# PathologyFoundation/plip

Measured on NVIDIA H100. Metric: image-text pairs/sec (224x224, 77-tok), higher is better.
Workload: dtype bf16

## Files before the change

include/plip_b200.h:

```cpp
#ifndef PLIP_B200_H_
#define PLIP_B200_H_

#include <stdint.h>

#ifdef __cplusplus
extern "C" {
#endif

#define PLIP_API __attribute__((visibility("default")))

#define PLIP_B200_ABI_VERSION 5

#define PLIP_IMAGE_SIZE 224
#define PLIP_EMBED_DIM 512
#define PLIP_TEXT_SEQ 77
#define PLIP_VOCAB 49408

typedef struct plip_engine plip_engine_t;

enum plip_pixel_format {
  PLIP_PIX_F32_NCHW = 0,
  PLIP_PIX_BF16_NCHW = 1,
  PLIP_PIX_U8_NHWC = 2
};
// ... 130 lines not shown

typedef struct plip_densenet plip_densenet_t;
PLIP_API int plip_densenet_num_tensors(void);
PLIP_API int plip_densenet_tensor_info(int index, plip_tensor_info_t* info);
PLIP_API uint64_t plip_densenet_blob_bytes(void);
PLIP_API uint64_t plip_densenet_workspace_bytes(int max_micro_batch);
PLIP_API int plip_densenet_create(const void* host_blob, uint64_t blob_bytes, int device, int max_micro_batch,
                                  plip_densenet_t** out);
PLIP_API int plip_densenet_destroy(plip_densenet_t* e);
PLIP_API int plip_densenet_max_micro_batch(const plip_densenet_t* e);
PLIP_API int plip_densenet_encode(plip_densenet_t* e, const void* tiles_dev, int64_t n, float* out_dev, void* stream);

PLIP_API int plip_encode_images_host(plip_engine_t* e, const void* pixels_host, int pixel_format, int64_t n,
                                     float* out_host, int normalize);
PLIP_API int plip_encode_text_host(plip_engine_t* e, const void* ids_host, int ids_dtype,
                                   const void* attention_mask_host, int64_t n, int seq_len,
                                   float* out_host, int normalize);

typedef struct plip_kernel_time {
  char name[48];
  int32_t launches;
  float total_ms;
  double flops;
  double bytes;
} plip_kernel_time_t;
PLIP_API int plip_profile_enable(plip_engine_t* e, int on);
PLIP_API int plip_profile_read(plip_engine_t* e, plip_kernel_time_t* out, int cap, int* count);

PLIP_API int plip_dbg_set_operand_format(int operand_format);
PLIP_API int plip_dbg_gemm(const void* A_bf16, int lda, const void* W_bf16, int ldw, int M, int N, int K,
                           const float* bias, void* out, int ldo, const float* pos, int epilogue, int cluster_size,
                           int block_n, const float* colsum, const float* stats_in, int n_partials, void* xb_out,
                           float* stats_out, void* stream);
PLIP_API int plip_dbg_resize_filter(int in_size, int out_size, int xx, int32_t* k_host, int k_cap, int* xmin,
                                    int* count);
PLIP_API int plip_dbg_resize_filter_bilinear(int in_size, int out_size, int xx, int32_t* k_host, int k_cap, int* xmin,
                                             int* count);
PLIP_API int plip_dbg_text_bucket_plan(const int32_t* lens_host, int64_t n, int seq_len, int32_t* perm_host,
                                       int32_t* bucket_start_host, int32_t* bucket_prefix_host, int cap);
PLIP_API int plip_dbg_rowstats_cast(const float* x, int64_t rows, int dim, void* xb_bf16, float* stats, void* stream);
PLIP_API int plip_dbg_layernorm(const float* x, int64_t rows, int dim, int64_t in_row_stride,
                                const float* gamma, const float* beta, float* out_f32, void* out_bf16,
                                void* stream);
PLIP_API int plip_dbg_attention(const void* qkv_bf16, int64_t n_seq, int seq_len, int heads, int causal,
                                const int32_t* key_mask, void* out_bf16, void* stream);
PLIP_API int plip_dbg_attention_probs(const void* qkv_bf16, int64_t n_seq, int seq_len, int heads, int causal,
                                      const int32_t* key_mask, float* probs_dev, void* stream);
PLIP_API int plip_dbg_densenet_op(int op, const void* in_dev, int lda, int64_t n, int side, int c_in, const void* w_dev,
                                  const float* a_scale, const float* a_shift, const float* e_scale,
                                  const float* e_shift, void* out_dev, int ldo, void* stream);
PLIP_API int plip_dbg_im2col(const void* pixels, int pixel_format, int64_t n, void* out_bf16, void* stream);
PLIP_API int plip_dbg_pos_interp(const float* pos_dev, int grid_h, int grid_w, float* out_dev, void* stream);
PLIP_API int plip_dbg_hidden_states_hw(plip_engine_t* e, const void* pixels_dev, int pixel_format, int64_t n,
                                       int height, int width, int num_layers, float* hidden_dev, void* stream);
PLIP_API int plip_dbg_hidden_states(plip_engine_t* e, int tower, const void* input_dev, int input_format,
                                    const void* attention_mask_dev, int64_t n, int num_layers,
                                    float* hidden_dev, void* stream);

#ifdef __cplusplus
}
#endif
#endif
```

plip_b200/_lib.py:

```python
from __future__ import annotations

import ctypes as C
from pathlib import Path

_PKG = Path(__file__).resolve().parent
LIB_PATH = _PKG / "libplip_b200.so"

_vp = C.c_void_p
_i = C.c_int
_i64 = C.c_int64
_u64 = C.c_uint64
_f = C.c_float
_fp = C.c_void_p


class TensorInfo(C.Structure):

    _fields_ = [
        ("name", C.c_char * 96),
        ("offset", C.c_uint64),
        ("numel", C.c_uint64),
        ("dtype", C.c_int32),
        ("rows", C.c_int32),
        ("cols", C.c_int32),
# ... 22 lines not shown

class WarpDesc(C.Structure):

    _fields_ = [("affine", C.c_double * 6), ("perspective", C.c_double * 8), ("flip", C.c_int32),
                ("apply_perspective", C.c_int32), ("fill", C.c_int32), ("reserved", C.c_int32)]


class SgdProblem(C.Structure):

    _fields_ = [("alpha", C.c_double), ("pos_weight", C.c_double), ("neg_weight", C.c_double), ("pos_class", C.c_int32),
                ("sigma_index", C.c_int32)]


class TowerOutputs(C.Structure):

    _fields_ = [("embeds", C.c_void_p), ("pooled", C.c_void_p), ("last_hidden", C.c_void_p), ("hidden", C.c_void_p),
                ("attn", C.c_void_p), ("normalize", C.c_int32)]


SIGNATURES = {
    "plip_last_error": (C.c_char_p, []),
    "plip_abi_version": (_i, []),
    "plip_launch_count": (_u64, []),
    "plip_weights_num_tensors": (_i, []),
    "plip_weights_tensor_info": (_i, [_i, C.POINTER(TensorInfo)]),
    "plip_weights_blob_bytes": (_u64, []),
    "plip_create": (_i, [_vp, _u64, _f, _i, _i, C.POINTER(_vp)]),
    "plip_create_ex": (_i, [_vp, _u64, _f, _i, _i, _i, C.POINTER(_vp)]),
    "plip_operand_format": (_i, [_vp]),
    "plip_set_text_pooling": (_i, [_vp, _i]),
    "plip_set_last_layer_pruning": (_i, [_vp, _i]),
    "plip_last_layer_pruning": (_i, [_vp]),
    "plip_dbg_set_operand_format": (_i, [_i]),
    "plip_destroy": (_i, [_vp]),
    "plip_workspace_bytes": (_u64, [_i]),
    "plip_logit_scale_exp": (_f, [_vp]),
    "plip_max_micro_batch": (_i, [_vp]),
    "plip_encode_images": (_i, [_vp, _vp, _i, _i64, _fp, _i, _vp]),
    "plip_encode_images_hw": (_i, [_vp, _vp, _i, _i64, _i, _i, _fp, _i, _vp]),
    "plip_encode_windows": (_i, [_vp, _vp, _i, _i, _i64, _vp, _i64, _fp, _i, _vp]),
    "plip_window_background_counts": (_i, [_vp, _i, _i, _i64, _vp, _i64, _i, _vp, _vp]),
    "plip_encode_text": (_i, [_vp, _vp, _i, _vp, _i64, _i, _fp, _i, _vp]),
    "plip_encode_text_prefix": (_i, [_vp, _vp, _i, _vp, _i64, _i, _i, _fp, _i, _vp]),
    "plip_vision_outputs": (_i, [_vp, _vp, _i, _i64, _i, _i, C.POINTER(TowerOutputs), _vp]),
    "plip_text_outputs": (_i, [_vp, _vp, _i, _vp, _i64, _i, C.POINTER(TowerOutputs), _vp]),
    "plip_similarity": (_i, [_fp, _i64, _fp, _i64, _f, _i, _i, _fp, _i64, _vp]),
    "plip_similarity_topk": (_i, [_fp, _i64, _fp, _i64, _f, _i, _i, _i, _vp, _fp, _vp]),
    "plip_l2_normalize": (_i, [_fp, _i64, _i, _vp]),
    "plip_window_mask_counts": (_i, [_vp, _i, _i, _i, _i64, _vp, _i64, _i, _vp, _vp]),
    "plip_resize_crop_u8": (_i, [_vp, _u64, _vp, _i64, _vp, _vp]),
    "plip_resize_crop_bilinear_u8": (_i, [_vp, _u64, _vp, _i64, _vp, _vp]),
    "plip_warp_tiles_u8": (_i, [_vp, _vp, _vp, _i64, _vp]),
    "plip_resize_region_workspace": (_i, [_i, _i, _i, _i, _i, _i, C.POINTER(_u64)]),
    "plip_resize_region_u8": (_i, [_vp, _i64, _i, _i, _i, _i, _vp, _i64, _i, _i, _i, _i, _vp, _u64, _vp]),
    "plip_resize_filter_bounds": (_i, [_i, _i, _vp]),
    "plip_sgd_shuffle_permutation": (_i, [_i64, C.c_uint32, _vp]),
    "plip_sgd_workspace_bytes": (_i, [_i64, _i, _i, C.POINTER(_u64)]),
    "plip_sgd_fit": (_i, [_fp, _i64, _i, _vp, _i, _vp, _i, _vp, _i, _i, C.c_double, _i, _fp, _vp, _vp, _vp, _vp, _u64,
                          _vp]),
    "plip_linear_decision": (_i, [_fp, _i64, _i, _fp, _vp, _i, _fp, _vp, _vp]),
    "plip_densenet_num_tensors": (_i, []),
    "plip_densenet_tensor_info": (_i, [_i, C.POINTER(TensorInfo)]),
    "plip_densenet_blob_bytes": (_u64, []),
    "plip_densenet_workspace_bytes": (_u64, [_i]),
    "plip_densenet_create": (_i, [_vp, _u64, _i, _i, C.POINTER(_vp)]),
    "plip_densenet_destroy": (_i, [_vp]),
# ... 58 lines not shown
```

plip_b200/csrc/engine.cu:

```cuda
#include "kernels.cuh"

#include <stdlib.h>
#include <string.h>

#include <array>
#include <map>
#include <string>
#include <tuple>
#include <vector>

namespace plip {
const char* get_last_error();

namespace {

struct Spec {
  std::string name;
  int dtype;
  int rows, cols, fused;
  uint64_t offset, numel;
};

void add(std::vector<Spec>& v, const std::string& name, int dtype, int rows, int cols, int fused = 0) {
  Spec s;
// ... 1216 lines not shown
  }
  for (int k = 0; k < nb; ++k) {
    const int64_t r0 = start[k], cnt = start[k + 1] - start[k];
    if (cnt <= 0) continue;
    if (int rc = plip_encode_text_prefix(e, d_ids + (size_t)r0 * row_bytes, ids_dtype,
                                         d_mask ? d_mask + (size_t)r0 * row_bytes : nullptr, cnt, seq_len, prefix[k],
                                         e->d_out + r0 * kProj, normalize, e->s_compute)) return rc;
  }
  std::vector<float> tmp((size_t)n * kProj);
  PLIP_CUDA_CHECK(cudaMemcpyAsync(tmp.data(), e->d_out, (size_t)n * kProj * 4, cudaMemcpyDeviceToHost, e->s_compute));
  PLIP_CUDA_CHECK(cudaStreamSynchronize(e->s_compute));
  for (int64_t i = 0; i < n; ++i)
    memcpy(out_host + (size_t)perm[(size_t)i] * kProj, tmp.data() + (size_t)i * kProj, (size_t)kProj * 4);
  return 0;
}

PLIP_API int plip_dbg_text_bucket_plan(const int32_t* lens_host, int64_t n, int seq_len, int32_t* perm_host,
                                       int32_t* bucket_start_host, int32_t* bucket_prefix_host, int cap) {
  if (!lens_host || !bucket_start_host || !bucket_prefix_host || n <= 0 || seq_len < 1 || seq_len > kTxtSeq || cap < 1) {
    set_last_error("plip_dbg_text_bucket_plan: bad argument");
    return -2;
  }
  return plan_text_buckets(lens_host, n, seq_len, perm_host, bucket_start_host, bucket_prefix_host, cap);
}

static int g_dbg_f16 = 0;
PLIP_API int plip_dbg_set_operand_format(int operand_format) {
  PLIP_REQUIRE(operand_format == PLIP_OPERAND_BF16 || operand_format == PLIP_OPERAND_FP16,
               "plip_dbg_set_operand_format: unknown operand format %d", operand_format);
  g_dbg_f16 = operand_format == PLIP_OPERAND_FP16 ? 1 : 0;
  return 0;
}

PLIP_API int plip_dbg_gemm(const void* A_bf16, int lda, const void* W_bf16, int ldw, int M, int N, int K,
                           const float* bias, void* out, int ldo, const float* pos, int epilogue, int cluster_size,
                           int block_n, const float* colsum, const float* stats_in, int n_partials, void* xb_out,
                           float* stats_out, void* stream) {
  GemmArgs g;
  g.A = static_cast<const __nv_bfloat16*>(A_bf16); g.lda = lda;
  g.W = static_cast<const __nv_bfloat16*>(W_bf16); g.ldw = ldw;
  g.M = M; g.N = N; g.K = K;
  g.bias = bias; g.out = out; g.ldo = ldo; g.pos = pos; g.epi = epilogue;
  g.colsum = colsum; g.stats_in = reinterpret_cast<const float2*>(stats_in); g.n_partials = n_partials;
  g.xb_out = static_cast<__nv_bfloat16*>(xb_out); g.stats_out = reinterpret_cast<float2*>(stats_out);
  g.force_cg = cluster_size; g.force_bn = block_n;
  g.f16 = g_dbg_f16;
  return launch_gemm(g, static_cast<cudaStream_t>(stream));
}

PLIP_API int plip_dbg_rowstats_cast(const float* x, int64_t rows, int dim, void* xb_bf16, float* stats, void* stream) {
  return launch_rowstats_cast(x, rows, dim, static_cast<__nv_bfloat16*>(xb_bf16), reinterpret_cast<float2*>(stats),
                              g_dbg_f16, static_cast<cudaStream_t>(stream));
}

PLIP_API int plip_dbg_layernorm(const float* x, int64_t rows, int dim, int64_t in_row_stride, const float* gamma,
                                const float* beta, float* out_f32, void* out_bf16, void* stream) {
  return launch_layernorm(x, nullptr, in_row_stride, rows, dim, gamma, beta, out_f32,
                          static_cast<__nv_bfloat16*>(out_bf16), g_dbg_f16, static_cast<cudaStream_t>(stream));
}

PLIP_API int plip_dbg_attention(const void* qkv_bf16, int64_t n_seq, int seq_len, int heads, int causal,
                                const int32_t* key_mask, void* out_bf16, void* stream) {
  return launch_attention(static_cast<const __nv_bfloat16*>(qkv_bf16), n_seq, seq_len, heads, causal != 0, key_mask,
                          static_cast<__nv_bfloat16*>(out_bf16), g_dbg_f16, static_cast<cudaStream_t>(stream));
}

PLIP_API int plip_dbg_attention_probs(const void* qkv_bf16, int64_t n_seq, int seq_len, int heads, int causal,
                                      const int32_t* key_mask, float* probs_dev, void* stream) {
  return launch_attention_probs(static_cast<const __nv_bfloat16*>(qkv_bf16), n_seq, seq_len, heads, causal != 0,
                                key_mask, probs_dev, g_dbg_f16, static_cast<cudaStream_t>(stream));
}

PLIP_API int plip_dbg_im2col(const void* pixels, int pixel_format, int64_t n, void* out_bf16, void* stream) {
  return launch_im2col(pixels, pixel_format, n, kImage, kImage, static_cast<__nv_bfloat16*>(out_bf16), g_dbg_f16,
                       static_cast<cudaStream_t>(stream));
}

PLIP_API int plip_dbg_pos_interp(const float* pos_dev, int grid_h, int grid_w, float* out_dev, void* stream) {
// ... 18 lines not shown
```

plip_b200/csrc/gemm.cuh:

```cuda
#pragma once
#include "common.cuh"

namespace plip {

enum GemmEpilogue : int {
  EPI_BIAS_BF16 = 0,
  EPI_BIAS_GELU_BF16 = 1,
  EPI_BIAS_RESID_F32 = 2,
  EPI_PATCH_F32 = 3,
  EPI_F32 = 4,
  EPI_LN_BIAS_BF16 = 5,
  EPI_LN_BIAS_GELU_BF16 = 6,
  EPI_NULL = 7,
  EPI_SIM_F32 = 8,
  EPI_COUNT = 9
};

constexpr int kStatSlots = 8;

struct GemmArgs {
  const __nv_bfloat16* A = nullptr;
  int lda = 0;
  const __nv_bfloat16* W = nullptr;
  int ldw = 0;
  int M = 0, N = 0, K = 0;
  const float* bias = nullptr;
  const float* rowscale = nullptr;
  void* out = nullptr;
  int ldo = 0;
  const float* pos = nullptr;
  int patches = kPatches;
  int seq = kVisSeq;
  const float* colsum = nullptr;
  const float2* stats_in = nullptr;
  int n_partials = 0;
  __nv_bfloat16* xb_out = nullptr;
  float2* stats_out = nullptr;
  int* n_tiles_used = nullptr;
  int epi = EPI_F32;
  int f16 = 0;
  int force_cg = 0;
  int force_bn = 0;
};

int launch_gemm(const GemmArgs& g, cudaStream_t stream);

}
```

plip_b200/csrc/gemm_wgmma.cu:

```cuda
#include "gemm.cuh"
#include "wgmma.cuh"

#include <stdio.h>
#include <stdlib.h>

namespace plip {

namespace {

constexpr int BM = 64;
constexpr int BK = 64;
constexpr int kThreads = 288;
constexpr int kConsumerWarps = 8;
constexpr uint32_t A_STAGE = BM * BK * 2;
constexpr uint32_t kStoreStageBytes = 16 * 128;

constexpr int x_boxes(int BN, int EPI) {
  return EPI != EPI_BIAS_RESID_F32 ? 2 : BN == 192 ? 3 : 2;
}

template <int BN, int EPI>
struct Cfg {
  static constexpr uint32_t B_STAGE = BN * BK * 2;
  static constexpr uint32_t STAGE = A_STAGE + B_STAGE;
  static constexpr int XBOXES = x_boxes(BN, EPI);
  static constexpr uint32_t EPI_BYTES = kConsumerWarps * XBOXES * kStoreStageBytes;
  static constexpr uint32_t BAR_BYTES = EPI == EPI_BIAS_RESID_F32 ? 512 : 256;
  static constexpr uint32_t ALIGN_SLACK = 1024;
  static constexpr int kMaxStages = (227 * 1024 - BAR_BYTES - EPI_BYTES - ALIGN_SLACK) / STAGE;
  static constexpr int STAGES = kMaxStages > 8 ? 8 : kMaxStages;
  static constexpr uint32_t SMEM_BYTES = STAGES * STAGE + EPI_BYTES + BAR_BYTES + ALIGN_SLACK;
};

struct GemmDev {
  int M, N, K;
  const float* bias;
  const float* rowscale;
  void* out;
  int ldo;
  const float* pos;
  int patches, seq;
  const float* colsum;
  const float2* stats_in;
  int n_partials;
  __nv_bfloat16* xb_out;
  float2* stats_out;
};

template <bool F16, int BN>
__device__ __forceinline__ void wgmma_ss(float (&d)[BN / 2], uint64_t adesc, uint64_t bdesc, uint32_t scale_d) {
  if constexpr (BN == 128) wgmma_ss_n128<F16>(d, adesc, bdesc, scale_d);
  else if constexpr (BN == 192) wgmma_ss_n192<F16>(d, adesc, bdesc, scale_d);
  else wgmma_ss_n256<F16>(d, adesc, bdesc, scale_d);
}

__device__ __forceinline__ float2 ln_row_terms(const GemmDev& p, int grow) {
  float s1 = 0.f, s2 = 0.f;
#pragma unroll
  for (int j = 0; j < kStatSlots; ++j) {
    const float2 t = (grow < p.M && j < p.n_partials) ? __ldg(p.stats_in + static_cast<size_t>(grow) * kStatSlots + j)
                                                      : make_float2(0.f, 0.f);
    s1 += t.x;
    s2 += t.y;
  }
  const float inv_k = 1.0f / static_cast<float>(p.K);
  const float mean = s1 * inv_k;
  const float rstd = rsqrtf(fmaxf(s2 * inv_k - mean * mean, 0.f) + kLnEps);
  return make_float2(-rstd * mean, rstd);
}

template <int BN, int EPI, bool F16>
__device__ __forceinline__ void epilogue_warp(const GemmDev& p, const CUtensorMap* tmC, float (&d)[BN / 2], uint32_t stage_smem,
                                              uint32_t& stage_sel, uint32_t xbar, int row_base, int col_base, int n_blk, int lane,
                                              float2 ln0, float2 ln1) {
  constexpr bool LN_FOLD = (EPI == EPI_LN_BIAS_BF16 || EPI == EPI_LN_BIAS_GELU_BF16);
  constexpr bool GELU = (EPI == EPI_BIAS_GELU_BF16 || EPI == EPI_LN_BIAS_GELU_BF16);
  constexpr bool HAS_BIAS = (EPI == EPI_BIAS_BF16 || EPI == EPI_BIAS_GELU_BF16 || EPI == EPI_BIAS_RESID_F32 || LN_FOLD);
  constexpr bool OUT_BF16 = (EPI == EPI_BIAS_BF16 || EPI == EPI_BIAS_GELU_BF16 || LN_FOLD);
  const int q = lane & 3, rr = lane >> 2;
  const int row0 = row_base + rr, row1 = row0 + 8;

  if constexpr (EPI == EPI_NULL) {
    float acc = 0.f;
#pragma unroll
    for (int i = 0; i < BN / 2; ++i) acc += d[i];
    if (acc == 1.2345e30f && p.M < 0) reinterpret_cast<float*>(p.out)[0] = acc;
  } else if constexpr (OUT_BF16) {
#pragma unroll
    for (int blk = 0; blk < BN / 64; ++blk) {
      const uint32_t buf = stage_smem + (stage_sel & 1u) * kStoreStageBytes;
      ++stage_sel;
      if (lane == 0) tma_store_wait_read_but_one();
      __syncwarp();
#pragma unroll
      for (int jj = 0; jj < 8; ++jj) {
        const int j = blk * 8 + jj;
        const int col = col_base + 8 * j + 2 * q;
        const float2 b = __ldg(reinterpret_cast<const float2*>(p.bias + col));
        float v00 = d[4 * j + 0], v01 = d[4 * j + 1], v10 = d[4 * j + 2], v11 = d[4 * j + 3];
        if constexpr (LN_FOLD) {
          const float2 cs = __ldg(reinterpret_cast<const float2*>(p.colsum + col));
          v00 = fmaf(ln0.y, v00, fmaf(ln0.x, cs.x, b.x));
          v01 = fmaf(ln0.y, v01, fmaf(ln0.x, cs.y, b.y));
          v10 = fmaf(ln1.y, v10, fmaf(ln1.x, cs.x, b.x));
          v11 = fmaf(ln1.y, v11, fmaf(ln1.x, cs.y, b.y));
        } else {
          v00 += b.x; v01 += b.y; v10 += b.x; v11 += b.y;
        }
        if constexpr (GELU) {
          v00 = quick_gelu(v00); v01 = quick_gelu(v01); v10 = quick_gelu(v10); v11 = quick_gelu(v11);
        }
        st_shared_b32(buf + rr * 128 + ((jj ^ rr) << 4) + q * 4, pack_op2<F16>(v00, v01));
        st_shared_b32(buf + (rr + 8) * 128 + ((jj ^ rr) << 4) + q * 4, pack_op2<F16>(v10, v11));
      }
      fence_proxy_async_smem();
      __syncwarp();
      if (lane == 0) {
        tma_store_2d(tmC, buf, col_base + blk * 64, row_base);
        tma_store_commit();
      }
    }
  } else if constexpr (EPI == EPI_BIAS_RESID_F32) {
    constexpr int kChunkCols = 32;
    constexpr int kChunks = BN / kChunkCols;
    constexpr int NB = x_boxes(BN, EPI);
    static_assert(kChunks % NB == 0, "every tile must start at staging block 0");
    constexpr int kUses = kChunks / NB;
    const bool ok0 = row0 < p.M, ok1 = row1 < p.M;
    const bool emit = p.xb_out != nullptr;
    const size_t o0 = static_cast<size_t>(ok0 ? row0 : 0) * p.ldo + col_base + 2 * q;
    const size_t o1 = o0 + 8 * static_cast<size_t>(p.ldo);
    uint32_t ph0 = 0;
    if constexpr (kUses % 2 != 0) ph0 = stage_sel++ & 1u;
    auto fetch = [&](int c) {
      if (lane == 0) {
        const uint32_t bar = xbar + 8u * (c % NB);
        mbar_arrive_expect_tx(bar, kStoreStageBytes);
        tma_load_2d(stage_smem + (c % NB) * kStoreStageBytes, tmC, bar, 2 * (col_base + c * kChunkCols), row_base);
      }
    };
    if (lane == 0) tma_store_wait_read();
    __syncwarp();
#pragma unroll
    for (int c = 0; c < NB; ++c) fetch(c);
    float st[2][2] = {};
#pragma unroll
    for (int c = 0; c < kChunks; ++c) {
      const int h = c < kChunks / 2 ? 0 : 1;
      mbar_wait(xbar + 8u * (c % NB), ph0 ^ ((c / NB) & 1u));
      const uint32_t buf = stage_smem + (c % NB) * kStoreStageBytes;
#pragma unroll
      for (int jj = 0; jj < kChunkCols / 8; ++jj) {
        const int j = c * (kChunkCols / 8) + jj;
        const int col = col_base + 8 * j + 2 * q;
        const uint32_t xoff = (((2 * jj + (q >> 1)) ^ rr) << 4) + (q & 1) * 8;
        const float2 b = __ldg(reinterpret_cast<const float2*>(p.bias + col));
        const float2 v0 = make_float2(d[4 * j + 0] + b.x, d[4 * j + 1] + b.y);
        const float2 v1 = make_float2(d[4 * j + 2] + b.x, d[4 * j + 3] + b.y);
// ... 61 lines not shown
      o1 = static_cast<size_t>(b1 * p.seq + 1 + (r1 - b1 * p.patches)) * p.ldo;
      q0 = static_cast<size_t>(1 + (r0 - b0 * p.patches)) * p.N;
      q1 = static_cast<size_t>(1 + (r1 - b1 * p.patches)) * p.N;
    }
#pragma unroll
    for (int j = 0; j < BN / 8; ++j) {
      const int col = col_base + 8 * j + 2 * q;
      float2 v0 = make_float2(d[4 * j + 0], d[4 * j + 1]), v1 = make_float2(d[4 * j + 2], d[4 * j + 3]);
      if constexpr (HAS_BIAS) {
        const float2 b = __ldg(reinterpret_cast<const float2*>(p.bias + col));
        v0.x += b.x; v0.y += b.y; v1.x += b.x; v1.y += b.y;
      }
      if constexpr (EPI == EPI_SIM_F32) {
        const float2 cs = __ldg(reinterpret_cast<const float2*>(p.bias + col));
        if (ok0) *reinterpret_cast<float2*>(out + o0 + col) = make_float2(v0.x * rs0 * cs.x, v0.y * rs0 * cs.y);
        if (ok1) *reinterpret_cast<float2*>(out + o1 + col) = make_float2(v1.x * rs1 * cs.x, v1.y * rs1 * cs.y);
      } else if constexpr (EPI == EPI_PATCH_F32) {
        if (ok0) {
          const float2 e = __ldg(reinterpret_cast<const float2*>(p.pos + q0 + col));
          *reinterpret_cast<float2*>(out + o0 + col) = make_float2(v0.x + e.x, v0.y + e.y);
        }
        if (ok1) {
          const float2 e = __ldg(reinterpret_cast<const float2*>(p.pos + q1 + col));
          *reinterpret_cast<float2*>(out + o1 + col) = make_float2(v1.x + e.x, v1.y + e.y);
        }
      } else {
        if (ok0) *reinterpret_cast<float2*>(out + o0 + col) = v0;
        if (ok1) *reinterpret_cast<float2*>(out + o1 + col) = v1;
      }
    }
  }
}

template <int CG, int BN, int EPI, bool F16>
__global__ void __launch_bounds__(kThreads, 1)
gemm_kernel(const __grid_constant__ CUtensorMap tmA, const __grid_constant__ CUtensorMap tmB,
            const __grid_constant__ CUtensorMap tmC, const GemmDev p) {
  using C = Cfg<BN, EPI>;
  constexpr int STAGES = C::STAGES;
  extern __shared__ uint8_t smem_raw[];
  const uint32_t smem_base = (smem_u32(smem_raw) + 1023u) & ~1023u;
  const uint32_t epi_base = smem_base + STAGES * C::STAGE;
  const uint32_t bar_base = epi_base + C::EPI_BYTES;
  auto full_bar = [&](int s) { return bar_base + 8u * s; };
  auto empty_bar = [&](int s) { return bar_base + 8u * (STAGES + s); };
  const uint32_t resid_bar = bar_base + 8u * (2 * STAGES);
  static_assert(8 * (2 * STAGES + (EPI == EPI_BIAS_RESID_F32 ? C::XBOXES * kConsumerWarps : 0)) <= C::BAR_BYTES,
                "barrier area too small");

  const int warp = threadIdx.x >> 5;
  const int lane = threadIdx.x & 31;
  const int wg = warp >> 2;
  const uint32_t cta_rank = (CG > 1) ? cluster_ctarank() : 0u;

  if (threadIdx.x == 0) {
    tma_prefetch_desc(&tmA);
    tma_prefetch_desc(&tmB);
    for (int s = 0; s < STAGES; ++s) {
      mbar_init(full_bar(s), 1);
      mbar_init(empty_bar(s), CG);
    }
    if constexpr (EPI == EPI_BIAS_RESID_F32) {
      tma_prefetch_desc(&tmC);
      for (int i = 0; i < C::XBOXES * kConsumerWarps; ++i) mbar_init(resid_bar + 8u * i, 1);
    }
    fence_mbar_init();
  }
  if constexpr (CG > 1) cluster_sync_all(); else __syncthreads();

  const int num_n_blk = p.N / BN;
  const int num_m_blk = (p.M + BM * CG - 1) / (BM * CG);
  const int num_tiles = num_m_blk * num_n_blk;
  const int num_kb = p.K / BK;
  const int tile0 = blockIdx.x / CG;
  const int tile_step = gridDim.x / CG;
  const int my_tiles = (num_tiles - tile0 + tile_step - 1) / tile_step;

  if (wg == 2) {
    if (lane == 0) {
      int s = 0;
      uint32_t ph = 0;
      for (int t = tile0; t < num_tiles; t += tile_step) {
        const int m0 = ((t / num_n_blk) * CG + cta_rank) * BM;
        const int n0 = (t % num_n_blk) * BN;
        for (int kb = 0; kb < num_kb; ++kb) {
          mbar_wait(empty_bar(s), ph ^ 1u);
          const uint32_t sa = smem_base + s * C::STAGE;
          const uint32_t sb = sa + A_STAGE;
          mbar_arrive_expect_tx(full_bar(s), C::STAGE);
          tma_load_2d(sa, &tmA, full_bar(s), kb * BK, m0);
          if constexpr (CG == 1) {
            tma_load_2d(sb, &tmB, full_bar(s), kb * BK, n0);
          } else {
            tma_load_2d_mc(sb + cta_rank * (C::B_STAGE / 2), &tmB, full_bar(s), kb * BK, n0 + cta_rank * (BN / 2), 0x3);
          }
          if (++s == STAGES) { s = 0; ph ^= 1u; }
        }
      }
    }
    __syncwarp();
  } else {
    const int wtid = threadIdx.x & 127;
    auto release = [&](int s) {
      if (wtid == 0) mbar_arrive(empty_bar(s));
      if constexpr (CG > 1) {
        if (wtid == 32) mbar_arrive_cluster(mapa_shared(empty_bar(s), cta_rank ^ 1u));
      }
    };
    float d[BN / 2];
    int s = 0;
    uint32_t ph = 0;
    auto skip_tile = [&]() {
      s += num_kb;
      ph ^= static_cast<uint32_t>(s / STAGES) & 1u;
      s %= STAGES;
    };
    uint32_t stage_sel = 0;
    const uint32_t my_turn = 1u + wg, other_turn = 2u - wg;
    const int rounds = (my_tiles + 1) / 2;
    if (wg == 1) skip_tile();
    for (int r = 0; r < rounds; ++r) {
      const int i = 2 * r + wg;
      const int t = tile0 + i * tile_step;
      const int n_blk = t % num_n_blk;
      const int m0 = ((t / num_n_blk) * CG + cta_rank) * BM;
      const int wrow = m0 + (warp & 3) * 16;
      float2 ln0 = make_float2(0.f, 1.f), ln1 = make_float2(0.f, 1.f);
      if constexpr (EPI == EPI_LN_BIAS_BF16 || EPI == EPI_LN_BIAS_GELU_BF16) {
        if (i < my_tiles) {
          ln0 = ln_row_terms(p, wrow + (lane >> 2));
          ln1 = ln_row_terms(p, wrow + (lane >> 2) + 8);
        }
      }
      if (wg == 1 || r > 0) named_barrier_sync<256>(my_turn);
      if (i >= my_tiles) break;
      int prev = -1;
      for (int kb = 0; kb < num_kb; ++kb) {
        mbar_wait(full_bar(s), ph);
        const uint32_t sa = smem_base + s * C::STAGE;
        const uint64_t adesc = make_smem_desc_sw128(sa, 1024, 16);
        const uint64_t bdesc = make_smem_desc_sw128(sa + A_STAGE, 1024, 16);
        wgmma_pin(d);
        wgmma_fence();
#pragma unroll
        for (int k = 0; k < BK / 16; ++k) wgmma_ss<F16, BN>(d, adesc + 2 * k, bdesc + 2 * k, (kb | k) != 0 ? 1u : 0u);
        wgmma_commit();
        wgmma_wait<1>();
        if (prev >= 0) release(prev);
        prev = s;
        if (++s == STAGES) { s = 0; ph ^= 1u; }
      }
      if (wg == 0 || r + 1 < rounds) named_barrier_arrive<256>(other_turn);
      wgmma_wait<0>();
      wgmma_pin(d);
      release(prev);
      skip_tile();
      epilogue_warp<BN, EPI, F16>(p, &tmC, d, epi_base + warp * C::XBOXES * kStoreStageBytes, stage_sel,
                                  resid_bar + 8u * C::XBOXES * warp, wrow,
                                  n_blk * BN, n_blk, lane, ln0, ln1);
    }
    if (lane == 0) tma_store_wait_all();
    __syncwarp();
  }
  if constexpr (CG > 1) cluster_sync_all();
}

int env_int(const char* name, int dflt) {
  const char* v = getenv(name);
  return v ? atoi(v) : dflt;
}

template <int CG, int BN, int EPI, bool F16>
int launch_inst(const GemmArgs& g, cudaStream_t stream) {
  using C = Cfg<BN, EPI>;
  auto kern = gemm_kernel<CG, BN, EPI, F16>;
  static unsigned long long configured = 0;
  static int max_groups = 0;
  if (first_use_on_device(configured)) {
    PLIP_CUDA_CHECK(cudaFuncSetAttribute(kern, cudaFuncAttributeMaxDynamicSharedMemorySize, (int)C::SMEM_BYTES));
    int dev = 0, sms = 0;
    PLIP_CUDA_CHECK(cudaGetDevice(&dev));
    PLIP_CUDA_CHECK(cudaDeviceGetAttribute(&sms, cudaDevAttrMultiProcessorCount, dev));
    max_groups = sms / CG;
    if (CG >= 2) {
      cudaLaunchConfig_t q = {};
      q.gridDim = dim3(sms / CG * CG);
      q.blockDim = dim3(kThreads);
      q.dynamicSmemBytes = C::SMEM_BYTES;
      cudaLaunchAttribute qa[1];
      qa[0].id = cudaLaunchAttributeClusterDimension;
      qa[0].val.clusterDim.x = CG; qa[0].val.clusterDim.y = 1; qa[0].val.clusterDim.z = 1;
      q.attrs = qa; q.numAttrs = 1;
      int n_clusters = 0;
      PLIP_CUDA_CHECK(cudaOccupancyMaxActiveClusters(&n_clusters, kern, &q));
      if (n_clusters > 0 && n_clusters < max_groups) max_groups = n_clusters;
    }
    PLIP_REQUIRE(max_groups > 0, "launch_gemm: no resident CTA fits (cg=%d bn=%d)", CG, BN);
  }
  CUtensorMap tmA, tmB;
  if (int rc = make_tmap_bf16_2d(&tmA, g.A, g.M, g.K, (uint64_t)g.lda * 2, BM, BK)) return rc;
  if (int rc = make_tmap_bf16_2d(&tmB, g.W, g.N, g.K, (uint64_t)g.ldw * 2, BN / CG, BK)) return rc;
  constexpr bool kOutBf16 = (EPI == EPI_BIAS_BF16 || EPI == EPI_BIAS_GELU_BF16 || EPI == EPI_LN_BIAS_BF16 ||
                             EPI == EPI_LN_BIAS_GELU_BF16);
  CUtensorMap tmC = tmA;
  if (kOutBf16)
    if (int rc = make_tmap_bf16_2d(&tmC, g.out, g.M, g.N, (uint64_t)g.ldo * 2, 16, 64)) return rc;
  if (EPI == EPI_BIAS_RESID_F32)
    if (int rc = make_tmap_bf16_2d(&tmC, g.out, g.M, 2 * (uint64_t)g.N, (uint64_t)g.ldo * 4, 16, 64)) return rc;

  GemmDev p;
  p.M = g.M; p.N = g.N; p.K = g.K;
  p.bias = g.bias; p.rowscale = g.rowscale; p.out = g.out; p.ldo = g.ldo; p.pos = g.pos;
  p.patches = g.patches; p.seq = g.seq;
  p.colsum = g.colsum; p.stats_in = g.stats_in; p.n_partials = g.n_partials;
  p.xb_out = g.xb_out; p.stats_out = g.stats_out;
  if (g.n_tiles_used) *g.n_tiles_used = 2 * (g.N / BN);

  const int num_tiles = ((g.M + BM * CG - 1) / (BM * CG)) * (g.N / BN);
  const int groups = max_groups < num_tiles ? max_groups : num_tiles;
  PLIP_CUDA_CHECK(launch_kernel(kern, dim3(groups * CG), dim3(kThreads), C::SMEM_BYTES, stream, CG, tmA, tmB, tmC, p));
  return 0;
}

template <int CG, int BN, bool F16>
int launch_epi_fmt(const GemmArgs& g, cudaStream_t stream) {
  switch (g.epi) {
    case EPI_BIAS_BF16: return launch_inst<CG, BN, EPI_BIAS_BF16, F16>(g, stream);
    case EPI_BIAS_GELU_BF16: return launch_inst<CG, BN, EPI_BIAS_GELU_BF16, F16>(g, stream);
    case EPI_BIAS_RESID_F32: return launch_inst<CG, BN, EPI_BIAS_RESID_F32, F16>(g, stream);
    case EPI_PATCH_F32: return launch_inst<CG, BN, EPI_PATCH_F32, F16>(g, stream);
    case EPI_F32: return launch_inst<CG, BN, EPI_F32, F16>(g, stream);
    case EPI_LN_BIAS_BF16: return launch_inst<CG, BN, EPI_LN_BIAS_BF16, F16>(g, stream);
    case EPI_LN_BIAS_GELU_BF16: return launch_inst<CG, BN, EPI_LN_BIAS_GELU_BF16, F16>(g, stream);
    case EPI_NULL: return launch_inst<CG, BN, EPI_NULL, F16>(g, stream);
    case EPI_SIM_F32: return launch_inst<CG, BN, EPI_SIM_F32, F16>(g, stream);
    default: set_last_error("launch_gemm: bad epilogue %d", g.epi); return -2;
  }
}
template <int CG, int BN>
int launch_epi(const GemmArgs& g, cudaStream_t stream) {
  return g.f16 ? launch_epi_fmt<CG, BN, true>(g, stream) : launch_epi_fmt<CG, BN, false>(g, stream);
}

}

int launch_gemm(const GemmArgs& g, cudaStream_t stream) {
  PLIP_REQUIRE(g.M > 0 && g.N > 0 && g.K > 0, "launch_gemm: empty problem M=%d N=%d K=%d", g.M, g.N, g.K);
  PLIP_REQUIRE(g.K % BK == 0, "launch_gemm: K=%d must be a multiple of %d", g.K, BK);
  PLIP_REQUIRE(g.N % 128 == 0 || g.N % 192 == 0, "launch_gemm: N=%d must be a multiple of 128 or 192", g.N);
  PLIP_REQUIRE((g.lda % 8) == 0 && (g.ldw % 8) == 0 && (g.ldo % 8) == 0,
               "launch_gemm: leading dimensions must be multiples of 8 elements");
  PLIP_REQUIRE((reinterpret_cast<uintptr_t>(g.A) & 15) == 0 && (reinterpret_cast<uintptr_t>(g.W) & 15) == 0 &&
               (reinterpret_cast<uintptr_t>(g.out) & 15) == 0,
               "launch_gemm: operands must be 16-byte aligned");
  if (g.epi == EPI_LN_BIAS_BF16 || g.epi == EPI_LN_BIAS_GELU_BF16)
    PLIP_REQUIRE(g.colsum && g.stats_in && g.bias && g.n_partials >= 1 && g.n_partials <= kStatSlots,
                 "launch_gemm: LayerNorm-folded epilogue needs colsum, stats and 1..%d partials", kStatSlots);
  if (g.epi == EPI_SIM_F32)
    PLIP_REQUIRE(g.bias && g.rowscale, "launch_gemm: the similarity epilogue needs row and column scales");
  if (g.epi == EPI_PATCH_F32)
    PLIP_REQUIRE(g.patches >= 1 && g.seq == g.patches + 1, "launch_gemm: patch epilogue with %d patches, %d rows",
                 g.patches, g.seq);
  if (g.xb_out || g.stats_out)
    PLIP_REQUIRE(g.epi == EPI_BIAS_RESID_F32 && g.xb_out && g.stats_out,
                 "launch_gemm: xb/stats outputs belong to the residual epilogue");
  static const int env_cg = env_int("PLIP_GEMM_CG", 0);
  static const int env_bn = env_int("PLIP_GEMM_BN", 0);
  int cg = g.force_cg ? g.force_cg : (env_cg ? env_cg : 2);
  int bn = g.force_bn ? g.force_bn : (env_bn ? env_bn : 256);
  if (g.N % bn != 0) bn = 128;
  if (!g.force_bn && g.stats_out && 2 * (g.N / bn) > kStatSlots && g.N % 256 == 0) bn = 256;
  PLIP_REQUIRE((cg == 1 || cg == 2) && (bn == 128 || bn == 256 || (bn == 192 && cg == 2)),
               "launch_gemm: bad config cg=%d bn=%d", cg, bn);
  PLIP_REQUIRE(!g.stats_out || 2 * (g.N / bn) <= kStatSlots, "launch_gemm: N=%d / BN=%d exceeds %d statistics slots",
               g.N, bn, kStatSlots);
  if (cg == 1) return bn == 256 ? launch_epi<1, 256>(g, stream) : launch_epi<1, 128>(g, stream);
  if (bn == 192) return launch_epi<2, 192>(g, stream);
  return bn == 256 ? launch_epi<2, 256>(g, stream) : launch_epi<2, 128>(g, stream);
}

}
```

Before: 27000.

## Add cooperative GEMM schedule with shared 128-row tiles and smem-staged epilogue params

Adds a cooperative warp-specialized schedule in which both consumer warpgroups split one 2*BM-row tile instead of alternating ping-pong tiles. In this mode bias and colsum are prefetched into shared memory with cp.async, and all TMA stores are drained together. By default it is chosen only for fp32-output epilogues (patch, plain f32, similarity, null), and only when there are enough tiles to fill the resident CTAs. The aim is better tensor-core utilization and less wait between tiles on those GEMMs, at the cost of losing the epilogue/mainloop overlap and adding an extra named barrier.

```diff
diff --git a/include/plip_b200.h b/include/plip_b200.h
--- a/include/plip_b200.h
+++ b/include/plip_b200.h
@@ -186,6 +186,7 @@
                            const float* bias, void* out, int ldo, const float* pos, int epilogue, int cluster_size,
                            int block_n, const float* colsum, const float* stats_in, int n_partials, void* xb_out,
                            float* stats_out, void* stream);
+PLIP_API int plip_dbg_set_gemm_schedule(int schedule);
 PLIP_API int plip_dbg_resize_filter(int in_size, int out_size, int xx, int32_t* k_host, int k_cap, int* xmin,
                                     int* count);
 PLIP_API int plip_dbg_resize_filter_bilinear(int in_size, int out_size, int xx, int32_t* k_host, int k_cap, int* xmin,
diff --git a/plip_b200/_lib.py b/plip_b200/_lib.py
--- a/plip_b200/_lib.py
+++ b/plip_b200/_lib.py
@@ -78,6 +78,7 @@
     "plip_set_last_layer_pruning": (_i, [_vp, _i]),
     "plip_last_layer_pruning": (_i, [_vp]),
     "plip_dbg_set_operand_format": (_i, [_i]),
+    "plip_dbg_set_gemm_schedule": (_i, [_i]),
     "plip_destroy": (_i, [_vp]),
     "plip_workspace_bytes": (_u64, [_i]),
     "plip_logit_scale_exp": (_f, [_vp]),
diff --git a/plip_b200/csrc/engine.cu b/plip_b200/csrc/engine.cu
--- a/plip_b200/csrc/engine.cu
+++ b/plip_b200/csrc/engine.cu
@@ -1272,6 +1272,14 @@
   return 0;
 }
 
+static int g_dbg_gemm_sched = 0;
+PLIP_API int plip_dbg_set_gemm_schedule(int schedule) {
+  PLIP_REQUIRE(schedule == 0 || schedule == kGemmPingPong || schedule == kGemmCooperative,
+               "plip_dbg_set_gemm_schedule: unknown schedule %d", schedule);
+  g_dbg_gemm_sched = schedule;
+  return 0;
+}
+
 PLIP_API int plip_dbg_gemm(const void* A_bf16, int lda, const void* W_bf16, int ldw, int M, int N, int K,
                            const float* bias, void* out, int ldo, const float* pos, int epilogue, int cluster_size,
                            int block_n, const float* colsum, const float* stats_in, int n_partials, void* xb_out,
@@ -1283,7 +1291,7 @@
   g.bias = bias; g.out = out; g.ldo = ldo; g.pos = pos; g.epi = epilogue;
   g.colsum = colsum; g.stats_in = reinterpret_cast<const float2*>(stats_in); g.n_partials = n_partials;
   g.xb_out = static_cast<__nv_bfloat16*>(xb_out); g.stats_out = reinterpret_cast<float2*>(stats_out);
-  g.force_cg = cluster_size; g.force_bn = block_n;
+  g.force_cg = cluster_size; g.force_bn = block_n; g.force_sched = g_dbg_gemm_sched;
   g.f16 = g_dbg_f16;
   return launch_gemm(g, static_cast<cudaStream_t>(stream));
 }
diff --git a/plip_b200/csrc/gemm.cuh b/plip_b200/csrc/gemm.cuh
--- a/plip_b200/csrc/gemm.cuh
+++ b/plip_b200/csrc/gemm.cuh
@@ -15,6 +15,8 @@
   EPI_SIM_F32 = 8,
   EPI_COUNT = 9
 };
+
+enum GemmSchedule : int { kGemmPingPong = 1, kGemmCooperative = 2 };
 
 constexpr int kStatSlots = 8;
 
@@ -41,6 +43,7 @@
   int f16 = 0;
   int force_cg = 0;
   int force_bn = 0;
+  int force_sched = 0;
 };
 
 int launch_gemm(const GemmArgs& g, cudaStream_t stream);
diff --git a/plip_b200/csrc/gemm_wgmma.cu b/plip_b200/csrc/gemm_wgmma.cu
--- a/plip_b200/csrc/gemm_wgmma.cu
+++ b/plip_b200/csrc/gemm_wgmma.cu
@@ -12,24 +12,30 @@
 constexpr int BK = 64;
 constexpr int kThreads = 288;
 constexpr int kConsumerWarps = 8;
-constexpr uint32_t A_STAGE = BM * BK * 2;
 constexpr uint32_t kStoreStageBytes = 16 * 128;
 
-constexpr int x_boxes(int BN, int EPI) {
-  return EPI != EPI_BIAS_RESID_F32 ? 2 : BN == 192 ? 3 : 2;
-}
-
-template <int BN, int EPI>
+constexpr int tile_rows(bool COOP) { return COOP ? 2 * BM : BM; }
+constexpr bool out_16bit(int EPI) {
+  return EPI == EPI_BIAS_BF16 || EPI == EPI_BIAS_GELU_BF16 || EPI == EPI_LN_BIAS_BF16 || EPI == EPI_LN_BIAS_GELU_BF16;
+}
+
+constexpr int x_boxes(int BN, int EPI, bool COOP) {
+  return COOP ? (out_16bit(EPI) ? BN / 64 : 0) : EPI != EPI_BIAS_RESID_F32 ? 2 : BN == 192 ? 3 : 2;
+}
+
+template <int BN, int EPI, bool COOP>
 struct Cfg {
+  static constexpr uint32_t A_STAGE = tile_rows(COOP) * BK * 2;
   static constexpr uint32_t B_STAGE = BN * BK * 2;
   static constexpr uint32_t STAGE = A_STAGE + B_STAGE;
-  static constexpr int XBOXES = x_boxes(BN, EPI);
+  static constexpr int XBOXES = x_boxes(BN, EPI, COOP);
   static constexpr uint32_t EPI_BYTES = kConsumerWarps * XBOXES * kStoreStageBytes;
+  static constexpr uint32_t PARAM_BYTES = COOP && out_16bit(EPI) ? 2 * 2 * BN * 4 : 0;
   static constexpr uint32_t BAR_BYTES = EPI == EPI_BIAS_RESID_F32 ? 512 : 256;
   static constexpr uint32_t ALIGN_SLACK = 1024;
-  static constexpr int kMaxStages = (227 * 1024 - BAR_BYTES - EPI_BYTES - ALIGN_SLACK) / STAGE;
+  static constexpr int kMaxStages = (227 * 1024 - BAR_BYTES - EPI_BYTES - PARAM_BYTES - ALIGN_SLACK) / STAGE;
   static constexpr int STAGES = kMaxStages > 8 ? 8 : kMaxStages;
-  static constexpr uint32_t SMEM_BYTES = STAGES * STAGE + EPI_BYTES + BAR_BYTES + ALIGN_SLACK;
+  static constexpr uint32_t SMEM_BYTES = STAGES * STAGE + EPI_BYTES + PARAM_BYTES + BAR_BYTES + ALIGN_SLACK;
 };
 
 struct GemmDev {
@@ -54,6 +60,12 @@
   else wgmma_ss_n256<F16>(d, adesc, bdesc, scale_d);
 }
 
+__device__ __forceinline__ void cp_async_8(uint32_t dst, const void* src) {
+  asm volatile("cp.async.ca.shared.global [%0], [%1], 8;" ::"r"(dst), "l"(src) : "memory");
+}
+__device__ __forceinline__ void cp_async_commit() { asm volatile("cp.async.commit_group;" ::: "memory"); }
+__device__ __forceinline__ void cp_async_wait_all() { asm volatile("cp.async.wait_group 0;" ::: "memory"); }
+
 __device__ __forceinline__ float2 ln_row_terms(const GemmDev& p, int grow) {
   float s1 = 0.f, s2 = 0.f;
 #pragma unroll
@@ -69,10 +81,10 @@
   return make_float2(-rstd * mean, rstd);
 }
 
-template <int BN, int EPI, bool F16>
+template <int BN, int EPI, bool F16, bool DRAIN>
 __device__ __forceinline__ void epilogue_warp(const GemmDev& p, const CUtensorMap* tmC, float (&d)[BN / 2], uint32_t stage_smem,
                                               uint32_t& stage_sel, uint32_t xbar, int row_base, int col_base, int n_blk, int lane,
-                                              float2 ln0, float2 ln1) {
+                                              float2 ln0, float2 ln1, const float* params = nullptr) {
   constexpr bool LN_FOLD = (EPI == EPI_LN_BIAS_BF16 || EPI == EPI_LN_BIAS_GELU_BF16);
   constexpr bool GELU = (EPI == EPI_BIAS_GELU_BF16 || EPI == EPI_LN_BIAS_GELU_BF16);
   constexpr bool HAS_BIAS = (EPI == EPI_BIAS_BF16 || EPI == EPI_BIAS_GELU_BF16 || EPI == EPI_BIAS_RESID_F32 || LN_FOLD);
@@ -86,44 +98,83 @@
     for (int i = 0; i < BN / 2; ++i) acc += d[i];
     if (acc == 1.2345e30f && p.M < 0) reinterpret_cast<float*>(p.out)[0] = acc;
   } else if constexpr (OUT_BF16) {
-#pragma unroll
-    for (int blk = 0; blk < BN / 64; ++blk) {
-      const uint32_t buf = stage_smem + (stage_sel & 1u) * kStoreStageBytes;
-      ++stage_sel;
-      if (lane == 0) tma_store_wait_read_but_one();
-      __syncwarp();
-#pragma unroll
-      for (int jj = 0; jj < 8; ++jj) {
-        const int j = blk * 8 + jj;
-        const int col = col_base + 8 * j + 2 * q;
-        const float2 b = __ldg(reinterpret_cast<const float2*>(p.bias + col));
-        float v00 = d[4 * j + 0], v01 = d[4 * j + 1], v10 = d[4 * j + 2], v11 = d[4 * j + 3];
-        if constexpr (LN_FOLD) {
-          const float2 cs = __ldg(reinterpret_cast<const float2*>(p.colsum + col));
-          v00 = fmaf(ln0.y, v00, fmaf(ln0.x, cs.x, b.x));
-          v01 = fmaf(ln0.y, v01, fmaf(ln0.x, cs.y, b.y));
-          v10 = fmaf(ln1.y, v10, fmaf(ln1.x, cs.x, b.x));
-          v11 = fmaf(ln1.y, v11, fmaf(ln1.x, cs.y, b.y));
-        } else {
-          v00 += b.x; v01 += b.y; v10 += b.x; v11 += b.y;
-        }
-        if constexpr (GELU) {
-          v00 = quick_gelu(v00); v01 = quick_gelu(v01); v10 = quick_gelu(v10); v11 = quick_gelu(v11);
-        }
-        st_shared_b32(buf + rr * 128 + ((jj ^ rr) << 4) + q * 4, pack_op2<F16>(v00, v01));
-        st_shared_b32(buf + (rr + 8) * 128 + ((jj ^ rr) << 4) + q * 4, pack_op2<F16>(v10, v11));
-      }
+    auto finish = [&](uint32_t buf, int j, int jj, float2 b, float2 cs) {
+      float v00 = d[4 * j + 0], v01 = d[4 * j + 1], v10 = d[4 * j + 2], v11 = d[4 * j + 3];
+      if constexpr (LN_FOLD) {
+        v00 = fmaf(ln0.y, v00, fmaf(ln0.x, cs.x, b.x));
+        v01 = fmaf(ln0.y, v01, fmaf(ln0.x, cs.y, b.y));
+        v10 = fmaf(ln1.y, v10, fmaf(ln1.x, cs.x, b.x));
+        v11 = fmaf(ln1.y, v11, fmaf(ln1.x, cs.y, b.y));
+      } else {
+        v00 += b.x; v01 += b.y; v10 += b.x; v11 += b.y;
+      }
+      if constexpr (GELU) {
+        v00 = quick_gelu(v00); v01 = quick_gelu(v01); v10 = quick_gelu(v10); v11 = quick_gelu(v11);
+      }
+      st_shared_b32(buf + rr * 128 + ((jj ^ rr) << 4) + q * 4, pack_op2<F16>(v00, v01));
+      st_shared_b32(buf + (rr + 8) * 128 + ((jj ^ rr) << 4) + q * 4, pack_op2<F16>(v10, v11));
+    };
+    auto stage_block = [&](uint32_t buf, int blk) {
+      if constexpr (DRAIN) {
+        constexpr int kGroup = 4;
+#pragma unroll
+        for (int g = 0; g < 8; g += kGroup) {
+          float2 b[kGroup], cs[kGroup];
+#pragma unroll
+          for (int i = 0; i < kGroup; ++i) {
+            const int c = 8 * (blk * 8 + g + i) + 2 * q;
+            b[i] = *reinterpret_cast<const float2*>(params + c);
+            cs[i] = LN_FOLD ? *reinterpret_cast<const float2*>(params + BN + c) : make_float2(0.f, 0.f);
+          }
+#pragma unroll
+          for (int i = 0; i < kGroup; ++i) finish(buf, blk * 8 + g + i, g + i, b[i], cs[i]);
+        }
+      } else {
+#pragma unroll
+        for (int jj = 0; jj < 8; ++jj) {
+          const int j = blk * 8 + jj;
+          const int col = col_base + 8 * j + 2 * q;
+          const float2 b = __ldg(reinterpret_cast<const float2*>(p.bias + col));
+          const float2 cs = LN_FOLD ? __ldg(reinterpret_cast<const float2*>(p.colsum + col)) : make_float2(0.f, 0.f);
+          finish(buf, j, jj, b, cs);
+        }
+      }
+    };
+    if constexpr (DRAIN) {
+      if (lane == 0) tma_store_wait_read();
+      cp_async_wait_all();
+      named_barrier_sync<256>(1u);
+#pragma unroll
+      for (int blk = 0; blk < BN / 64; ++blk) stage_block(stage_smem + blk * kStoreStageBytes, blk);
       fence_proxy_async_smem();
       __syncwarp();
       if (lane == 0) {
-        tma_store_2d(tmC, buf, col_base + blk * 64, row_base);
+#pragma unroll
+        for (int blk = 0; blk < BN / 64; ++blk)
+          tma_store_2d(tmC, stage_smem + blk * kStoreStageBytes, col_base + blk * 64, row_base);
         tma_store_commit();
+      }
+    } else {
+#pragma unroll
+      for (int blk = 0; blk < BN / 64; ++blk) {
+        const uint32_t buf = stage_smem + (stage_sel & 1u) * kStoreStageBytes;
+        ++stage_sel;
+        if (lane == 0) tma_store_wait_read_but_one();
+        __syncwarp();
+        stage_block(buf, blk);
+        fence_proxy_async_smem();
+        __syncwarp();
+        if (lane == 0) {
+          tma_store_2d(tmC, buf, col_base + blk * 64, row_base);
+          tma_store_commit();
+        }
       }
     }
   } else if constexpr (EPI == EPI_BIAS_RESID_F32) {
     constexpr int kChunkCols = 32;
     constexpr int kChunks = BN / kChunkCols;
-    constexpr int NB = x_boxes(BN, EPI);
+    static_assert(!DRAIN, "the residual epilogue runs in the ping-pong schedule only");
+    constexpr int NB = x_boxes(BN, EPI, false);
     static_assert(kChunks % NB == 0, "every tile must start at staging block 0");
     constexpr int kUses = kChunks / NB;
     const bool ok0 = row0 < p.M, ok1 = row1 < p.M;
@@ -251,16 +302,19 @@
   }
 }
 
-template <int CG, int BN, int EPI, bool F16>
+template <int CG, int BN, int EPI, bool F16, bool COOP>
 __global__ void __launch_bounds__(kThreads, 1)
 gemm_kernel(const __grid_constant__ CUtensorMap tmA, const __grid_constant__ CUtensorMap tmB,
             const __grid_constant__ CUtensorMap tmC, const GemmDev p) {
-  using C = Cfg<BN, EPI>;
+  using C = Cfg<BN, EPI, COOP>;
   constexpr int STAGES = C::STAGES;
+  constexpr int TM = tile_rows(COOP);
+  static_assert(!(COOP && EPI == EPI_BIAS_RESID_F32), "the residual epilogue needs the ping-pong overlap");
   extern __shared__ uint8_t smem_raw[];
   const uint32_t smem_base = (smem_u32(smem_raw) + 1023u) & ~1023u;
   const uint32_t epi_base = smem_base + STAGES * C::STAGE;
-  const uint32_t bar_base = epi_base + C::EPI_BYTES;
+  const uint32_t param_base = epi_base + C::EPI_BYTES;
+  const uint32_t bar_base = param_base + C::PARAM_BYTES;
   auto full_bar = [&](int s) { return bar_base + 8u * s; };
   auto empty_bar = [&](int s) { return bar_base + 8u * (STAGES + s); };
   const uint32_t resid_bar = bar_base + 8u * (2 * STAGES);
@@ -277,7 +331,7 @@
     tma_prefetch_desc(&tmB);
     for (int s = 0; s < STAGES; ++s) {
       mbar_init(full_bar(s), 1);
-      mbar_init(empty_bar(s), CG);
+      mbar_init(empty_bar(s), (COOP ? 2 : 1) * CG);
     }
     if constexpr (EPI == EPI_BIAS_RESID_F32) {
       tma_prefetch_desc(&tmC);
@@ -288,7 +342,7 @@
   if constexpr (CG > 1) cluster_sync_all(); else __syncthreads();
 
   const int num_n_blk = p.N / BN;
-  const int num_m_blk = (p.M + BM * CG - 1) / (BM * CG);
+  const int num_m_blk = (p.M + TM * CG - 1) / (TM * CG);
   const int num_tiles = num_m_blk * num_n_blk;
   const int num_kb = p.K / BK;
   const int tile0 = blockIdx.x / CG;
@@ -300,12 +354,12 @@
       int s = 0;
       uint32_t ph = 0;
       for (int t = tile0; t < num_tiles; t += tile_step) {
-        const int m0 = ((t / num_n_blk) * CG + cta_rank) * BM;
+        const int m0 = ((t / num_n_blk) * CG + cta_rank) * TM;
         const int n0 = (t % num_n_blk) * BN;
         for (int kb = 0; kb < num_kb; ++kb) {
           mbar_wait(empty_bar(s), ph ^ 1u);
           const uint32_t sa = smem_base + s * C::STAGE;
-          const uint32_t sb = sa + A_STAGE;
+          const uint32_t sb = sa + C::A_STAGE;
           mbar_arrive_expect_tx(full_bar(s), C::STAGE);
           tma_load_2d(sa, &tmA, full_bar(s), kb * BK, m0);
           if constexpr (CG == 1) {
@@ -329,36 +383,13 @@
     float d[BN / 2];
     int s = 0;
     uint32_t ph = 0;
-    auto skip_tile = [&]() {
-      s += num_kb;
-      ph ^= static_cast<uint32_t>(s / STAGES) & 1u;
-      s %= STAGES;
-    };
-    uint32_t stage_sel = 0;
-    const uint32_t my_turn = 1u + wg, other_turn = 2u - wg;
-    const int rounds = (my_tiles + 1) / 2;
-    if (wg == 1) skip_tile();
-    for (int r = 0; r < rounds; ++r) {
-      const int i = 2 * r + wg;
-      const int t = tile0 + i * tile_step;
-      const int n_blk = t % num_n_blk;
-      const int m0 = ((t / num_n_blk) * CG + cta_rank) * BM;
-      const int wrow = m0 + (warp & 3) * 16;
-      float2 ln0 = make_float2(0.f, 1.f), ln1 = make_float2(0.f, 1.f);
-      if constexpr (EPI == EPI_LN_BIAS_BF16 || EPI == EPI_LN_BIAS_GELU_BF16) {
-        if (i < my_tiles) {
-          ln0 = ln_row_terms(p, wrow + (lane >> 2));
-          ln1 = ln_row_terms(p, wrow + (lane >> 2) + 8);
-        }
-      }
-      if (wg == 1 || r > 0) named_barrier_sync<256>(my_turn);
-      if (i >= my_tiles) break;
+    auto main_loop = [&](uint32_t a_off) {
       int prev = -1;
       for (int kb = 0; kb < num_kb; ++kb) {
         mbar_wait(full_bar(s), ph);
         const uint32_t sa = smem_base + s * C::STAGE;
-        const uint64_t adesc = make_smem_desc_sw128(sa, 1024, 16);
-        const uint64_t bdesc = make_smem_desc_sw128(sa + A_STAGE, 1024, 16);
+        const uint64_t adesc = make_smem_desc_sw128(sa + a_off, 1024, 16);
+        const uint64_t bdesc = make_smem_desc_sw128(sa + C::A_STAGE, 1024, 16);
         wgmma_pin(d);
         wgmma_fence();
 #pragma unroll
@@ -369,14 +400,71 @@
         prev = s;
         if (++s == STAGES) { s = 0; ph ^= 1u; }
       }
-      if (wg == 0 || r + 1 < rounds) named_barrier_arrive<256>(other_turn);
-      wgmma_wait<0>();
-      wgmma_pin(d);
-      release(prev);
-      skip_tile();
-      epilogue_warp<BN, EPI, F16>(p, &tmC, d, epi_base + warp * C::XBOXES * kStoreStageBytes, stage_sel,
-                                  resid_bar + 8u * C::XBOXES * warp, wrow,
-                                  n_blk * BN, n_blk, lane, ln0, ln1);
+      return prev;
+    };
+    auto ln_terms = [&](int wrow, float2& ln0, float2& ln1) {
+      if constexpr (EPI == EPI_LN_BIAS_BF16 || EPI == EPI_LN_BIAS_GELU_BF16) {
+        ln0 = ln_row_terms(p, wrow + (lane >> 2));
+        ln1 = ln_row_terms(p, wrow + (lane >> 2) + 8);
+      }
+    };
+    if constexpr (COOP) {
+      uint32_t stage_sel = 0;
+      uint32_t param_buf = 0;
+      for (int t = tile0; t < num_tiles; t += tile_step) {
+        const int n_blk = t % num_n_blk;
+        const int m0 = ((t / num_n_blk) * CG + cta_rank) * TM;
+        const int wrow = m0 + wg * BM + (warp & 3) * 16;
+        const uint32_t params = param_base + param_buf * (2 * BN * 4);
+        if constexpr (C::PARAM_BYTES != 0) {
+          constexpr bool LN_FOLD = (EPI == EPI_LN_BIAS_BF16 || EPI == EPI_LN_BIAS_GELU_BF16);
+          static_assert(BN <= 2 * BM * 2, "one 8-byte piece of bias and of colsum per consumer thread");
+          const int c = threadIdx.x;
+          if (c < BN / 2) cp_async_8(params + c * 8, p.bias + n_blk * BN + 2 * c);
+          else if (LN_FOLD && c < BN) cp_async_8(params + BN * 4 + (c - BN / 2) * 8, p.colsum + n_blk * BN + 2 * (c - BN / 2));
+          cp_async_commit();
+          param_buf ^= 1u;
+        }
+        float2 ln0 = make_float2(0.f, 1.f), ln1 = make_float2(0.f, 1.f);
+        ln_terms(wrow, ln0, ln1);
+        const int prev = main_loop(static_cast<uint32_t>(wg) * (BM * BK * 2));
+        wgmma_wait<0>();
+        wgmma_pin(d);
+        release(prev);
+        epilogue_warp<BN, EPI, F16, true>(p, &tmC, d, epi_base + warp * C::XBOXES * kStoreStageBytes, stage_sel, 0u,
+                                          wrow, n_blk * BN, n_blk, lane, ln0, ln1,
+                                          reinterpret_cast<const float*>(smem_raw + (params - smem_u32(smem_raw))));
+      }
+    } else {
+      auto skip_tile = [&]() {
+        s += num_kb;
+        ph ^= static_cast<uint32_t>(s / STAGES) & 1u;
+        s %= STAGES;
+      };
+      uint32_t stage_sel = 0;
+      const uint32_t my_turn = 1u + wg, other_turn = 2u - wg;
+      const int rounds = (my_tiles + 1) / 2;
+      if (wg == 1) skip_tile();
+      for (int r = 0; r < rounds; ++r) {
+        const int i = 2 * r + wg;
+        const int t = tile0 + i * tile_step;
+        const int n_blk = t % num_n_blk;
+        const int m0 = ((t / num_n_blk) * CG + cta_rank) * TM;
+        const int wrow = m0 + (warp & 3) * 16;
+        float2 ln0 = make_float2(0.f, 1.f), ln1 = make_float2(0.f, 1.f);
+        if (i < my_tiles) ln_terms(wrow, ln0, ln1);
+        if (wg == 1 || r > 0) named_barrier_sync<256>(my_turn);
+        if (i >= my_tiles) break;
+        const int prev = main_loop(0u);
+        if (wg == 0 || r + 1 < rounds) named_barrier_arrive<256>(other_turn);
+        wgmma_wait<0>();
+        wgmma_pin(d);
+        release(prev);
+        skip_tile();
+        epilogue_warp<BN, EPI, F16, false>(p, &tmC, d, epi_base + warp * C::XBOXES * kStoreStageBytes, stage_sel,
+                                           resid_bar + 8u * C::XBOXES * warp, wrow,
+                                           n_blk * BN, n_blk, lane, ln0, ln1);
+      }
     }
     if (lane == 0) tma_store_wait_all();
     __syncwarp();
@@ -389,10 +477,10 @@
   return v ? atoi(v) : dflt;
 }
 
-template <int CG, int BN, int EPI, bool F16>
-int launch_inst(const GemmArgs& g, cudaStream_t stream) {
-  using C = Cfg<BN, EPI>;
-  auto kern = gemm_kernel<CG, BN, EPI, F16>;
+template <int CG, int BN, int EPI, bool F16, bool COOP>
+int resident_groups() {
+  using C = Cfg<BN, EPI, COOP>;
+  auto kern = gemm_kernel<CG, BN, EPI, F16, COOP>;
   static unsigned long long configured = 0;
   static int max_groups = 0;
   if (first_use_on_device(configured)) {
@@ -416,13 +504,20 @@
     }
     PLIP_REQUIRE(max_groups > 0, "launch_gemm: no resident CTA fits (cg=%d bn=%d)", CG, BN);
   }
+  return max_groups;
+}
+
+template <int CG, int BN, int EPI, bool F16, bool COOP>
+int launch_sched(const GemmArgs& g, cudaStream_t stream) {
+  using C = Cfg<BN, EPI, COOP>;
+  constexpr int TM = tile_rows(COOP);
+  const int max_groups = resident_groups<CG, BN, EPI, F16, COOP>();
+  if (max_groups <= 0) return max_groups < 0 ? max_groups : -2;
   CUtensorMap tmA, tmB;
-  if (int rc = make_tmap_bf16_2d(&tmA, g.A, g.M, g.K, (uint64_t)g.lda * 2, BM, BK)) return rc;
+  if (int rc = make_tmap_bf16_2d(&tmA, g.A, g.M, g.K, (uint64_t)g.lda * 2, TM, BK)) return rc;
   if (int rc = make_tmap_bf16_2d(&tmB, g.W, g.N, g.K, (uint64_t)g.ldw * 2, BN / CG, BK)) return rc;
-  constexpr bool kOutBf16 = (EPI == EPI_BIAS_BF16 || EPI == EPI_BIAS_GELU_BF16 || EPI == EPI_LN_BIAS_BF16 ||
-                             EPI == EPI_LN_BIAS_GELU_BF16);
   CUtensorMap tmC = tmA;
-  if (kOutBf16)
+  if (out_16bit(EPI))
     if (int rc = make_tmap_bf16_2d(&tmC, g.out, g.M, g.N, (uint64_t)g.ldo * 2, 16, 64)) return rc;
   if (EPI == EPI_BIAS_RESID_F32)
     if (int rc = make_tmap_bf16_2d(&tmC, g.out, g.M, 2 * (uint64_t)g.N, (uint64_t)g.ldo * 4, 16, 64)) return rc;
@@ -435,10 +530,28 @@
   p.xb_out = g.xb_out; p.stats_out = g.stats_out;
   if (g.n_tiles_used) *g.n_tiles_used = 2 * (g.N / BN);
 
-  const int num_tiles = ((g.M + BM * CG - 1) / (BM * CG)) * (g.N / BN);
+  const int num_tiles = ((g.M + TM * CG - 1) / (TM * CG)) * (g.N / BN);
   const int groups = max_groups < num_tiles ? max_groups : num_tiles;
-  PLIP_CUDA_CHECK(launch_kernel(kern, dim3(groups * CG), dim3(kThreads), C::SMEM_BYTES, stream, CG, tmA, tmB, tmC, p));
+  PLIP_CUDA_CHECK(launch_kernel(gemm_kernel<CG, BN, EPI, F16, COOP>, dim3(groups * CG), dim3(kThreads), C::SMEM_BYTES,
+                                stream, CG, tmA, tmB, tmC, p));
   return 0;
+}
+
+constexpr bool coop_by_default(int EPI) { return !out_16bit(EPI) && EPI != EPI_BIAS_RESID_F32; }
+
+template <int CG, int BN, int EPI, bool F16>
+int launch_inst(const GemmArgs& g, cudaStream_t stream) {
+  if constexpr (EPI == EPI_BIAS_RESID_F32) {
+    return launch_sched<CG, BN, EPI, F16, false>(g, stream);
+  } else {
+    bool coop = g.force_sched == kGemmCooperative;
+    if (g.force_sched == 0 && coop_by_default(EPI)) {
+      const int groups = resident_groups<CG, BN, EPI, F16, true>();
+      if (groups <= 0) return groups < 0 ? groups : -2;
+      coop = ((g.M + 2 * BM * CG - 1) / (2 * BM * CG)) * (g.N / BN) >= groups;
+    }
+    return coop ? launch_sched<CG, BN, EPI, F16, true>(g, stream) : launch_sched<CG, BN, EPI, F16, false>(g, stream);
+  }
 }
 
 template <int CG, int BN, bool F16>
@@ -483,6 +596,10 @@
   if (g.xb_out || g.stats_out)
     PLIP_REQUIRE(g.epi == EPI_BIAS_RESID_F32 && g.xb_out && g.stats_out,
                  "launch_gemm: xb/stats outputs belong to the residual epilogue");
+  PLIP_REQUIRE(g.force_sched == 0 || g.force_sched == kGemmPingPong || g.force_sched == kGemmCooperative,
+               "launch_gemm: unknown schedule %d", g.force_sched);
+  PLIP_REQUIRE(!(g.force_sched == kGemmCooperative && g.epi == EPI_BIAS_RESID_F32),
+               "launch_gemm: the residual epilogue runs in the ping-pong schedule only");
   static const int env_cg = env_int("PLIP_GEMM_CG", 0);
   static const int env_bn = env_int("PLIP_GEMM_BN", 0);
   int cg = g.force_cg ? g.force_cg : (env_cg ? env_cg : 2);
```

Result: no change. 26970, median of 6 (-0.1%).
